# izhengfan/se2lam

Measured on NVIDIA H100. Metric: ORB keypoints/sec at 640x480 (8-level pyramid, 1000 kps/frame), higher is better.
Workload: dtype u8

## Files before the change

se2lam_b200/csrc/fast_screen.h:

```cpp
#pragma once
#include <cstdint>

#if defined(__CUDACC__)
#define SE2_HD __host__ __device__ __forceinline__
#else
#define SE2_HD inline
#endif

namespace fastpx {
SE2_HD int16_t lo16(unsigned a) { return (int16_t)(a & 0xFFFF); }
SE2_HD int16_t hi16(unsigned a) { return (int16_t)(a >> 16); }
SE2_HD unsigned pack16(int lo, int hi) { return ((unsigned)lo & 0xFFFFu) | ((unsigned)hi << 16); }
SE2_HD unsigned perm(unsigned a, unsigned b, unsigned s) {
#if defined(__CUDA_ARCH__)
    return __byte_perm(a, b, s);
#else
    const uint64_t src = ((uint64_t)b << 32) | a;
    unsigned r = 0;
    for (int i = 0; i < 4; ++i) {
        const unsigned sel = (s >> (4 * i)) & 0xF;
        unsigned byte = (unsigned)(src >> (8 * (sel & 7))) & 0xFF;
        if (sel & 8) byte = (byte & 0x80) ? 0xFF : 0x00;
        r |= byte << (8 * i);
    }
    return r;
#endif
}
SE2_HD unsigned maxs2(unsigned a, unsigned b) {
#if defined(__CUDA_ARCH__)
    return __vmaxs2(a, b);
#else
    return pack16(lo16(a) > lo16(b) ? lo16(a) : lo16(b), hi16(a) > hi16(b) ? hi16(a) : hi16(b));
#endif
}
SE2_HD unsigned mins2(unsigned a, unsigned b) {
#if defined(__CUDA_ARCH__)
    return __vmins2(a, b);
#else
    return pack16(lo16(a) < lo16(b) ? lo16(a) : lo16(b), hi16(a) < hi16(b) ? hi16(a) : hi16(b));
#endif
}
SE2_HD unsigned min3s2(unsigned a, unsigned b, unsigned c) {
#if defined(__CUDA_ARCH__)
    return __vimin3_s16x2(a, b, c);
#else
    return mins2(mins2(a, b), c);
#endif
}
SE2_HD unsigned max3s2(unsigned a, unsigned b, unsigned c) {
#if defined(__CUDA_ARCH__)
    return __vimax3_s16x2(a, b, c);
#else
    return maxs2(maxs2(a, b), c);
#endif
}
SE2_HD unsigned add2(unsigned a, unsigned b) {
#if defined(__CUDA_ARCH__)
    return __vadd2(a, b);
#else
    return pack16((lo16(a) + lo16(b)) & 0xFFFF, (hi16(a) + hi16(b)) & 0xFFFF);
#endif
}
}

namespace fastpx {

SE2_HD unsigned screen_T1(int t) { return (unsigned)(0x10000 - (257 + t)) * 0x10001u; }
SE2_HD unsigned screen_U1(int t) { return (unsigned)(256 - t) * 0x10001u; }

SE2_HD unsigned screen4(unsigned n3, unsigned s3, unsigned n2l, unsigned n2c, unsigned n2r, unsigned s2l, unsigned s2c, unsigned s2r,
                        unsigned zl, unsigned zc, unsigned zr, unsigned T1, unsigned U1) {
    const unsigned w_m3 = perm(zl, zc, 0x4321), w_p3 = perm(zc, zr, 0x6543);
    const unsigned nw_ = perm(n2l, n2c, 0x5432), ne_ = perm(n2c, n2r, 0x5432);
    const unsigned sw_ = perm(s2l, s2c, 0x5432), se_ = perm(s2c, s2r, 0x5432);
    unsigned m = 0;
#if defined(__CUDA_ARCH__)
#pragma unroll
#endif
    for (int hlf = 0; hlf < 2; ++hlf) {
        const unsigned sel = hlf ? 0x4342u : 0x4140u;
        const unsigned cb = perm(zc, 0, sel) + 0x01000100u;
        const unsigned e0 = cb - perm(s3, 0, sel), e8 = cb - perm(n3, 0, sel);
        const unsigned e4 = cb - perm(w_p3, 0, sel), e12 = cb - perm(w_m3, 0, sel);
        const unsigned e2 = cb - perm(se_, 0, sel), e10 = cb - perm(nw_, 0, sel);
        const unsigned e6 = cb - perm(ne_, 0, sel), e14 = cb - perm(sw_, 0, sel);
        const unsigned D = mins2(min3s2(maxs2(e0, e8), maxs2(e4, e12), maxs2(e2, e10)), maxs2(e6, e14));
        const unsigned B = maxs2(max3s2(mins2(e0, e8), mins2(e4, e12), mins2(e2, e10)), mins2(e6, e14));
        const unsigned r = maxs2(add2(D, T1), add2(~B, U1));
        const unsigned ok = ~r & 0x80008000u;
        m |= ((ok >> 15) & 1u) << (2 * hlf) | ((ok >> 31) & 1u) << (2 * hlf + 1);
    }
    return m;
}

SE2_HD unsigned inside_mask8(int x0, int cw) {
    const int lo = x0 < 0 ? -x0 : 0;
    const int hi = cw - x0 < 8 ? cw - x0 : 8;
    return (0xFFu << lo) & (0xFFu >> (8 - hi)) & 0xFFu;
}

SE2_HD int first_group(int shift) { return (shift + 3) >> 2; }
SE2_HD int groups_per_row(int cw, int shift) { return ((shift + 2 + cw) >> 2) - first_group(shift) + 1; }
SE2_HD int group_x0(int g, int shift) { return 4 * (g + first_group(shift)) - 3 - shift; }
struct ItemWalk {
    int y, g, dY, dG, G;
    SE2_HD void init(int tid, int nthreads, int groups) { G = groups; y = tid / G; g = tid - y * G; dY = nthreads / G; dG = nthreads - dY * G; }
    SE2_HD void next() { g += dG; y += dY; if (g >= G) { g -= G; ++y; } }
};

}
```

se2lam_b200/csrc/orb.cu:

```cuda
#include <cuda.h>

#include <algorithm>
#include <cmath>
#include <cstring>
#include <vector>

#include "blur_px.h"
#include "common.h"
#include "fast_screen.h"
#include "introselect.h"

namespace {

using se2gpu::fail;

constexpr int EDGE = 16;
constexpr int HALF_PATCH = 15;
constexpr int PATCH = 31;
constexpr int MAX_LEVELS = 16;
constexpr int FAST_THREADS = 256;
constexpr int ORB_LANES = 4;
constexpr int BLUR_WARPS = 4;
constexpr int BLUR_TH = 48;

// ... 169 lines not shown
            rowinfo[tx] = r;
            rmin = r.s0; rmax = r.s1;
        }
#pragma unroll
        for (int o = 16; o > 0; o >>= 1) { rmin = min(rmin, __shfl_xor_sync(0xffffffffu, rmin, o)); rmax = max(rmax, __shfl_xor_sync(0xffffffffu, rmax, o)); }
        if (tx == 0) { s_lo[1] = rmin; s_hi[1] = rmax; }
    }
    __syncthreads();
    const int c_min = min(min(s_cmin[0], s_cmin[1]), min(s_cmin[2], s_cmin[3])), c_max = max(max(s_cmax[0], s_cmax[1]), max(s_cmax[2], s_cmax[3]));
    const int c_lo = c_min & ~15, nvec = c_max < 0 ? 0 : (c_max - c_lo) / 16 + 1;
    const int r_lo = s_lo[1], nsr = s_hi[1] - r_lo + 1;
    if (nsr > max_rows || nvec * 16 > raw_pitch) { if (tid == 0) *d.err = 3; return; }
    const uint8_t* src = d.plain + f * d.frame_plane_bytes + S.plane_off + (size_t)EDGE * S.pitch + EDGE;
    asm volatile("griddepcontrol.wait;" ::: "memory");
    if (nvec <= 16) {
        const int v = tid & 15;
        if (v < nvec)
            for (int r = tid >> 4; r < nsr; r += 16)
                *reinterpret_cast<uint4*>(raw + r * raw_pitch + 16 * v) = __ldg(reinterpret_cast<const uint4*>(src + (size_t)(r_lo + r) * S.pitch + c_lo) + v);
    } else {
        for (int i = tid; i < nsr * nvec; i += 256) {
            const int r = i / nvec, v = i - r * nvec;
            *reinterpret_cast<uint4*>(raw + r * raw_pitch + 16 * v) = __ldg(reinterpret_cast<const uint4*>(src + (size_t)(r_lo + r) * S.pitch + c_lo) + v);
        }
    }
    int sx0[4], sx1[4], a0[4], a1[4];
    unsigned vmask = 0;
#pragma unroll
    for (int q = 0; q < 4; ++q) {
        const ResizeCol c = colinfo[4 * tx + q];
        sx0[q] = c.valid ? c.sx0 - c_lo : 0; sx1[q] = c.valid ? c.sx1 - c_lo : 0;
        a0[q] = c.a0; a1[q] = c.a1;
        vmask |= c.valid ? (0xFFu << (8 * q)) : 0u;
    }
    __syncthreads();
    unsigned wq[4], selq[4];
    bool pairq[4];
    int w0 = 0;
    bool window_ok = true;
    {
        int mn = 0x7fffffff;
#pragma unroll
        for (int q = 0; q < 4; ++q) if ((vmask >> (8 * q)) & 1u) mn = min(mn, sx0[q]);
        if (mn == 0x7fffffff) mn = 0;
        w0 = mn >> 2;
#pragma unroll
        for (int q = 0; q < 4; ++q) {
            const bool valid = (vmask >> (8 * q)) & 1u;
            const int o = valid ? sx0[q] - 4 * w0 : 0;
            if (valid && (o + 1 > 11 || (sx1[q] != sx0[q] + 1 && a1[q] != 0))) window_ok = false;
            pairq[q] = o >= 7;
            const int o2 = o - (pairq[q] ? 4 : 0);
            selq[q] = (unsigned)o2 | ((unsigned)(o2 + 1) << 4);
            wq[q] = ((unsigned)a0[q] & 0xFFFFu) | ((unsigned)a1[q] << 16);
            if (a0[q] < 0 || a1[q] < 0) window_ok = false;
        }
    }
    if (x4 < W) {
        if (window_ok) {
            for (int r = ty; r < nsr; r += 8) {
                const uint32_t* rw = reinterpret_cast<const uint32_t*>(raw + r * raw_pitch) + w0;
                const uint32_t W0 = rw[0], W1 = rw[1], W2 = rw[2];
                unsigned hq[4];
#pragma unroll
                for (int q = 0; q < 4; ++q) {
                    const unsigned bytes = __byte_perm(pairq[q] ? W1 : W0, pairq[q] ? W2 : W1, selq[q]);
                    hq[q] = __dp2a_lo(wq[q], bytes, 0u) >> 4;
                }
                *reinterpret_cast<uint2*>(hbuf + r * 128 + 4 * tx) = make_uint2(hq[0] | (hq[1] << 16), hq[2] | (hq[3] << 16));
            }
        } else {
            for (int r = ty; r < nsr; r += 8) {
                const uint8_t* rp = raw + r * raw_pitch;
                const unsigned h0 = (unsigned)((rp[sx0[0]] * a0[0] + rp[sx1[0]] * a1[0]) >> 4), h1 = (unsigned)((rp[sx0[1]] * a0[1] + rp[sx1[1]] * a1[1]) >> 4);
                const unsigned h2 = (unsigned)((rp[sx0[2]] * a0[2] + rp[sx1[2]] * a1[2]) >> 4), h3 = (unsigned)((rp[sx0[3]] * a0[3] + rp[sx1[3]] * a1[3]) >> 4);
                *reinterpret_cast<uint2*>(hbuf + r * 128 + 4 * tx) = make_uint2((h0 & 0xFFFFu) | (h1 << 16), (h2 & 0xFFFFu) | (h3 << 16));
            }
        }
    }
    __syncthreads();
    if (x4 >= L.pitch) return;
    uint8_t* plane = d.plain + f * d.frame_plane_bytes + L.plane_off;
#pragma unroll
    for (int k = 0; k < RESIZE_TR / 8; ++k) {
        const int r = ty + 8 * k, y = y0 + r;
        if (y >= H) break;
        uint32_t word = 0;
        if (x4 < W) {
            const ResizeRow ri = rowinfo[r];
            const uint2 A = *reinterpret_cast<const uint2*>(hbuf + (ri.s0 - r_lo) * 128 + 4 * tx);
            const uint2 B = *reinterpret_cast<const uint2*>(hbuf + (ri.s1 - r_lo) * 128 + 4 * tx);
            const unsigned v0 = (unsigned)((((ri.b0 * (int)(A.x & 0xFFFFu)) >> 16) + ((ri.b1 * (int)(B.x & 0xFFFFu)) >> 16) + 2) >> 2);
            const unsigned v1 = (unsigned)((((ri.b0 * (int)(A.x >> 16)) >> 16) + ((ri.b1 * (int)(B.x >> 16)) >> 16) + 2) >> 2);
            const unsigned v2 = (unsigned)((((ri.b0 * (int)(A.y & 0xFFFFu)) >> 16) + ((ri.b1 * (int)(B.y & 0xFFFFu)) >> 16) + 2) >> 2);
            const unsigned v3 = (unsigned)((((ri.b0 * (int)(A.y >> 16)) >> 16) + ((ri.b1 * (int)(B.y >> 16)) >> 16) + 2) >> 2);
            word = (v0 | (v1 << 8) | (v2 << 16) | (v3 << 24)) & vmask;
        }
        *reinterpret_cast<uint32_t*>(plane + (size_t)y * L.pitch + x4) = word;
    }
}

__device__ __forceinline__ unsigned fast_cv(int v) { return (unsigned)(256 + v) | ((unsigned)(256 - v) << 16); }
__device__ __forceinline__ unsigned fast_q(unsigned p, unsigned cv) { return p * 0xFFFFu + cv; }

__device__ __forceinline__ int fast_arc_score(const uint8_t* __restrict__ p, int pw) {
    const unsigned cv = fast_cv(p[0]);
    unsigned q[16];
    q[0] = fast_q(p[3 * pw], cv);       q[1] = fast_q(p[3 * pw + 1], cv);   q[2] = fast_q(p[2 * pw + 2], cv);    q[3] = fast_q(p[pw + 3], cv);
    q[4] = fast_q(p[3], cv);            q[5] = fast_q(p[-pw + 3], cv);      q[6] = fast_q(p[-2 * pw + 2], cv);   q[7] = fast_q(p[-3 * pw + 1], cv);
    q[8] = fast_q(p[-3 * pw], cv);      q[9] = fast_q(p[-3 * pw - 1], cv);  q[10] = fast_q(p[-2 * pw - 2], cv);  q[11] = fast_q(p[-pw - 3], cv);
    q[12] = fast_q(p[-3], cv);          q[13] = fast_q(p[pw - 3], cv);      q[14] = fast_q(p[2 * pw - 2], cv);   q[15] = fast_q(p[3 * pw - 1], cv);
    unsigned m3[16];
#pragma unroll
    for (int k = 0; k < 16; ++k) m3[k] = __vimin3_s16x2(q[k], q[(k + 1) & 15], q[(k + 2) & 15]);
    unsigned best = 0;
#pragma unroll
    for (int k = 0; k < 16; k += 2) {
        const unsigned a9 = __vimin3_s16x2(m3[k], m3[(k + 3) & 15], m3[(k + 6) & 15]);
        const unsigned b9 = __vimin3_s16x2(m3[k + 1], m3[(k + 4) & 15], m3[(k + 7) & 15]);
        best = __vimax3_s16x2(best, a9, b9);
    }
    return (int)max(best & 0xFFFFu, best >> 16) - 256;
}

struct FastMaps { CUtensorMap m[MAX_LEVELS]; };
__device__ __forceinline__ unsigned orb_smem_u32(const void* p) { return (unsigned)__cvta_generic_to_shared(p); }
__device__ __forceinline__ void orb_mbar_init(unsigned long long* bar, unsigned count) {
    asm volatile("mbarrier.init.shared::cta.b64 [%0], %1;" ::"r"(orb_smem_u32(bar)), "r"(count) : "memory");
    asm volatile("fence.mbarrier_init.release.cluster;" ::: "memory");
}
__device__ __forceinline__ bool orb_mbar_wait(unsigned long long* bar, unsigned parity) {
    const long long t0 = clock64();
    for (;;) {
        unsigned done;
        asm volatile(
            "{\n"
            ".reg .pred p;\n"
            "mbarrier.try_wait.parity.shared::cta.b64 p, [%1], %2;\n"
            "selp.u32 %0, 1, 0, p;\n"
            "}\n" : "=r"(done) : "r"(orb_smem_u32(bar)), "r"(parity) : "memory");
        if (done) return true;
        if (clock64() - t0 > 400000000LL) return false;
    }
}
__device__ __forceinline__ void orb_tma_box3(void* dst_smem, const CUtensorMap* map, int x, int y, int z, unsigned bytes, unsigned long long* bar) {
    asm volatile("mbarrier.arrive.expect_tx.shared::cta.b64 _, [%0], %1;" ::"r"(orb_smem_u32(bar)), "r"(bytes) : "memory");
    asm volatile("cp.async.bulk.tensor.3d.shared::cluster.global.tile.mbarrier::complete_tx::bytes [%0], [%1, {%2, %3, %4}], [%5];"
                 ::"r"(orb_smem_u32(dst_smem)), "l"(map), "r"(x), "r"(y), "r"(z), "r"(orb_smem_u32(bar)) : "memory");
}

template <bool TMA>
__global__ void __launch_bounds__(FAST_THREADS, TMA ? 0 : 5) orb_fast_cells(OrbDev d, const __grid_constant__ FastMaps maps) {
    extern __shared__ __align__(128) uint8_t smem_raw[];
    __shared__ int s_total, s_ncand;
    __shared__ __align__(8) unsigned long long s_bar;
    const CellGeo c = d.cells[blockIdx.x];
    const int f = blockIdx.y + d.frame0;
    CellHdr* hdr = d.hdr + (size_t)f * d.n_cells + blockIdx.x;
    const int cw = c.x1 - c.x0, ch = c.y1 - c.y0;
    if (c.skipped || cw <= 0 || ch <= 0) {
        if (threadIdx.x == 0) { hdr->n_base = 0; hdr->n_a = 0; hdr->n_b = 0; }
        return;
    }
    const LevelGeo& L = d.levels[c.level];
    const int bx0 = c.x0 - 3 + EDGE, ax0 = bx0 & (TMA ? ~15 : ~3), shift = bx0 - ax0;
    const int pw = TMA ? L.fbw : (shift + cw + 6 + 3) & ~3, pww = pw >> 2;
    const int ph = TMA ? L.fbh : ch + 6;
    uint8_t* smem = TMA ? smem_raw + ((128u - (orb_smem_u32(smem_raw) & 127u)) & 127u) : smem_raw;
    const int nbits = pw * ch, nwords = (nbits + 31) >> 5;
    const int g0 = fastpx::first_group(shift), G = fastpx::groups_per_row(cw, shift), nitems = ch * G;
    uint8_t* patch = smem;
    uint8_t* score = smem + ((pw * ph + 15) & ~15);
    uint32_t* bitmap = reinterpret_cast<uint32_t*>(score + ((pw * (ch + 2) + 15) & ~15));
    uint32_t* woff = bitmap + nwords;
    uint16_t* list = reinterpret_cast<uint16_t*>(woff + nwords);
    if (TMA) {
        if (threadIdx.x == 0) orb_mbar_init(&s_bar, 1);
        __syncthreads();
        if (threadIdx.x == 0) orb_tma_box3(patch, &maps.m[c.level], ax0, c.y0 - 3 + EDGE, f, (unsigned)(pw * ph), &s_bar);
    } else {
        const uint8_t* plane = d.plain + f * d.frame_plane_bytes + L.plane_off;
        const int by0 = c.y0 - 3 + EDGE;
        for (int i = threadIdx.x; i < pww * ph; i += FAST_THREADS) {
            const int py = i / pww, pxw = i - py * pww;
            reinterpret_cast<uint32_t*>(patch)[i] = *reinterpret_cast<const uint32_t*>(plane + (size_t)(by0 + py) * L.pitch + ax0 + 4 * pxw);
        }
    }
    constexpr int NW = FAST_THREADS / 32;
    const int lane = threadIdx.x & 31, wid = threadIdx.x >> 5;
    const uint8_t* p0 = patch + 3 * pw + 3 + shift;
    fastpx::ItemWalk first;
    first.init((int)threadIdx.x, FAST_THREADS, G);
    int thr = d.fast_th;
    for (int pass = 0; pass < 2; ++pass) {
        for (int i = threadIdx.x; i < (pw * (ch + 2) + 3) / 4; i += FAST_THREADS) reinterpret_cast<uint32_t*>(score)[i] = 0u;
        for (int i = threadIdx.x; i < nwords; i += FAST_THREADS) bitmap[i] = 0u;
        if (threadIdx.x == 0) s_ncand = 0;
        if (TMA && pass == 0 && !orb_mbar_wait(&s_bar, 0)) { *d.err = 4; return; }
        __syncthreads();
        {
            const uint32_t* pwords = reinterpret_cast<const uint32_t*>(patch);
            const unsigned T1 = fastpx::screen_T1(thr), U1 = fastpx::screen_U1(thr);
            fastpx::ItemWalk it = first;
            for (int it0 = wid * 32; it0 < nitems; it0 += NW * 32) {
                unsigned m = 0;
                const int col0 = fastpx::group_x0(it.g, shift);
                if (it.y < ch) {
                    const uint32_t* c = pwords + (it.y + 3) * pww + it.g + g0;
                    const uint32_t n3 = c[-3 * pww], s3 = c[3 * pww];
                    const uint32_t n2a = c[-2 * pww - 1], n2b = c[-2 * pww], n2c = c[-2 * pww + 1];
                    const uint32_t s2a = c[2 * pww - 1], s2b = c[2 * pww], s2c = c[2 * pww + 1];
                    const uint32_t za = c[-1], zb = c[0], zc = c[1];
                    m = fastpx::screen4(n3, s3, n2a, n2b, n2c, s2a, s2b, s2c, za, zb, zc, T1, U1) & fastpx::inside_mask8(col0, cw) & 0xFu;
                }
                const int cnt = __popc(m);
                int inc = cnt;
#pragma unroll
                for (int o = 1; o < 32; o <<= 1) { const int u = __shfl_up_sync(0xffffffffu, inc, o); if (lane >= o) inc += u; }
                const int tot = __shfl_sync(0xffffffffu, inc, 31);
                if (tot) {
                    int base = 0;
                    if (lane == 31) base = atomicAdd(&s_ncand, tot);
                    base = __shfl_sync(0xffffffffu, base, 31) + inc - cnt;
                    const int e0 = it.y * pw + col0;
                    while (m) {
                        const int j = __ffs(m) - 1;
                        m &= m - 1;
                        list[base++] = (uint16_t)(e0 + j);
                    }
                }
                it.next();
            }
        }
        __syncthreads();
        const int ncand = s_ncand;
        for (int i = threadIdx.x; i < ncand; i += FAST_THREADS) {
            const int off = list[i];
            const int m = fast_arc_score(p0 + off, pw);
            if (m > thr) score[off + pw + 1] = (uint8_t)(m - 1);
        }
        __syncthreads();
        for (int i = threadIdx.x; i < ncand; i += FAST_THREADS) {
            const int off = list[i];
            const uint8_t* q = score + off + pw + 1;
            const int sc = q[0];
            if (sc && sc > q[-pw - 1] && sc > q[-pw] && sc > q[-pw + 1] && sc > q[-1] && sc > q[1] && sc > q[pw - 1] && sc > q[pw] && sc > q[pw + 1])
                atomicOr(&bitmap[off >> 5], 1u << (off & 31));
        }
        __syncthreads();
        if (wid == 0) {
            int run = 0;
            for (int b0 = 0; b0 < nwords; b0 += 32) {
                const int v = (b0 + lane < nwords) ? __popc(bitmap[b0 + lane]) : 0;
                int inc = v;
#pragma unroll
                for (int o = 1; o < 32; o <<= 1) { const int u = __shfl_up_sync(0xffffffffu, inc, o); if (lane >= o) inc += u; }
                if (b0 + lane < nwords) woff[b0 + lane] = run + inc - v;
                run += __shfl_sync(0xffffffffu, inc, 31);
            }
            if (lane == 0) s_total = run;
        }
        __syncthreads();
        if (s_total > 3 || thr == 7) break;
        thr = 7;
        __syncthreads();
    }
    uint32_t* out = d.cand + (size_t)f * d.cand_total + c.cand_off;
    for (int j = threadIdx.x; j < nwords; j += FAST_THREADS) {
        uint32_t w = bitmap[j];
        int pos = woff[j];
        while (w) {
            const int off = j * 32 + __ffs(w) - 1;
            w &= w - 1;
            const int y = off / pw, x = off - y * pw;
            if (pos < c.cand_cap) out[pos] = ((uint32_t)score[off + pw + 1] << 24) | ((uint32_t)(c.y0 + y) << 12) | (uint32_t)(c.x0 + x);
            else *d.err = 1;
            ++pos;
        }
    }
    if (threadIdx.x == 0) { hdr->n_base = s_total; hdr->n_a = s_total; hdr->n_b = s_total; }
}

__device__ __forceinline__ int fast_arc_score_qr(const uint8_t* __restrict__ p, int pw, int t) {
    const int v = p[0];
    const int c0 = v - p[3 * pw], c8 = v - p[-3 * pw];
    bool dk = (c0 > t) | (c8 > t), br = (c0 < -t) | (c8 < -t);
    if (!(dk | br)) return 0;
    const int c4 = v - p[3], c12 = v - p[-3];
    dk &= (c4 > t) | (c12 > t); br &= (c4 < -t) | (c12 < -t);
    if (!(dk | br)) return 0;
    const int c2 = v - p[2 * pw + 2], c10 = v - p[-2 * pw - 2];
    dk &= (c2 > t) | (c10 > t); br &= (c2 < -t) | (c10 < -t);
    if (!(dk | br)) return 0;
    const int c6 = v - p[-2 * pw + 2], c14 = v - p[2 * pw - 2];
    dk &= (c6 > t) | (c14 > t); br &= (c6 < -t) | (c14 < -t);
    if (!(dk | br)) return 0;
#define SE2_PK(dv) ((static_cast<unsigned>(dv) & 0xFFFFu) | (static_cast<unsigned>(-(dv)) << 16))
    unsigned q[16];
    q[0] = SE2_PK(c0);   q[1] = SE2_PK(v - p[3 * pw + 1]);    q[2] = SE2_PK(c2);    q[3] = SE2_PK(v - p[pw + 3]);
    q[4] = SE2_PK(c4);   q[5] = SE2_PK(v - p[-pw + 3]);       q[6] = SE2_PK(c6);    q[7] = SE2_PK(v - p[-3 * pw + 1]);
    q[8] = SE2_PK(c8);   q[9] = SE2_PK(v - p[-3 * pw - 1]);   q[10] = SE2_PK(c10);  q[11] = SE2_PK(v - p[-pw - 3]);
    q[12] = SE2_PK(c12); q[13] = SE2_PK(v - p[pw - 3]);       q[14] = SE2_PK(c14);  q[15] = SE2_PK(v - p[3 * pw - 1]);
#undef SE2_PK
    unsigned m3[16];
#pragma unroll
    for (int k = 0; k < 16; ++k) m3[k] = __vimin3_s16x2(q[k], q[(k + 1) & 15], q[(k + 2) & 15]);
    unsigned best = 0x80008000u;
#pragma unroll
    for (int k = 0; k < 16; k += 2) {
        const unsigned a9 = __vimin3_s16x2(m3[k], m3[(k + 3) & 15], m3[(k + 6) & 15]);
        const unsigned b9 = __vimin3_s16x2(m3[k + 1], m3[(k + 4) & 15], m3[(k + 7) & 15]);
        best = __vimax3_s16x2(best, a9, b9);
    }
    const int mdark = static_cast<short>(best & 0xFFFFu), mbright = static_cast<short>(best >> 16);
    return max(mdark, mbright);
}

__global__ void __launch_bounds__(FAST_THREADS) orb_fast_cells_big(OrbDev d) {
    extern __shared__ uint8_t smem[];
    __shared__ int s_total;
    const CellGeo c = d.cells[blockIdx.x];
    const int f = blockIdx.y + d.frame0;
    CellHdr* hdr = d.hdr + (size_t)f * d.n_cells + blockIdx.x;
    const int cw = c.x1 - c.x0, ch = c.y1 - c.y0;
    if (c.skipped || cw <= 0 || ch <= 0) {
        if (threadIdx.x == 0) { hdr->n_base = 0; hdr->n_a = 0; hdr->n_b = 0; }
        return;
    }
    const LevelGeo& L = d.levels[c.level];
    const uint8_t* plane = d.plain + f * d.frame_plane_bytes + L.plane_off;
    const int bx0 = c.x0 - 3 + EDGE, by0 = c.y0 - 3 + EDGE;
    const int ax0 = bx0 & ~3, shift = bx0 - ax0;
    const int ph = ch + 6, sw = cw + 2, sh = ch + 2;
    const int pww = (shift + cw + 6 + 3) >> 2, pw = pww * 4;
    uint8_t* patch = smem;
    uint8_t* score = smem + ((pw * ph + 15) & ~15);
    const int nseg = (cw + 31) >> 5, nchunk = ch * nseg;
    int* cnt = reinterpret_cast<int*>(score + ((sw * sh + 15) & ~15));
    for (int i = threadIdx.x; i < pww * ph; i += FAST_THREADS) {
        const int py = i / pww, pxw = i - py * pww;
        reinterpret_cast<uint32_t*>(patch)[i] = *reinterpret_cast<const uint32_t*>(plane + (size_t)(by0 + py) * L.pitch + ax0 + 4 * pxw);
    }
    constexpr int NW = FAST_THREADS / 32;
    const int lane = threadIdx.x & 31, wid = threadIdx.x >> 5;
    const uint8_t* p0 = patch + 3 * pw + 3 + shift;
    int thr = d.fast_th;
    unsigned long long keepmask = 0;
    for (int pass = 0; pass < 2; ++pass) {
        for (int i = threadIdx.x; i < (sw * sh + 3) / 4; i += FAST_THREADS) reinterpret_cast<uint32_t*>(score)[i] = 0u;
        __syncthreads();
        for (int cidx = wid; cidx < nchunk; cidx += NW) {
            const int y = cidx / nseg, x = (cidx - y * nseg) * 32 + lane;
            if (x < cw) {
                const int m = fast_arc_score_qr(p0 + y * pw + x, pw, thr);
                if (m > thr) score[(y + 1) * sw + (x + 1)] = (uint8_t)(m - 1);
            }
        }
        __syncthreads();
        keepmask = 0;
        int t = 0;
        for (int cidx = wid; cidx < nchunk; cidx += NW, ++t) {
            const int y = cidx / nseg, x = (cidx - y * nseg) * 32 + lane;
            bool keep = false;
            if (x < cw) {
                const uint8_t* q = score + (y + 1) * sw + (x + 1);
                const int s = q[0];
                if (s) keep = s > q[-sw - 1] && s > q[-sw] && s > q[-sw + 1] && s > q[-1] && s > q[1] && s > q[sw - 1] && s > q[sw] && s > q[sw + 1];
            }
            const unsigned bal = __ballot_sync(0xffffffffu, keep);
            if (lane == 0) cnt[cidx] = __popc(bal);
            if (keep && t < 64) keepmask |= 1ull << t;
        }
        __syncthreads();
        if (wid == 0) {
            int run = 0;
            for (int b0 = 0; b0 < nchunk; b0 += 32) {
                const int v = (b0 + lane < nchunk) ? cnt[b0 + lane] : 0;
                int inc = v;
#pragma unroll
                for (int o = 1; o < 32; o <<= 1) { const int u = __shfl_up_sync(0xffffffffu, inc, o); if (lane >= o) inc += u; }
                if (b0 + lane < nchunk) cnt[b0 + lane] = run + inc - v;
                run += __shfl_sync(0xffffffffu, inc, 31);
            }
            if (lane == 0) s_total = run;
        }
        __syncthreads();
        if (s_total > 3 || thr == 7) break;
        thr = 7;
        __syncthreads();
    }
    uint32_t* out = d.cand + (size_t)f * d.cand_total + c.cand_off;
    int t = 0;
    for (int cidx = wid; cidx < nchunk; cidx += NW, ++t) {
        const int y = cidx / nseg, x = (cidx - y * nseg) * 32 + lane;
        bool keep;
        int s = 0;
        if (t < 64) {
            keep = (keepmask >> t) & 1ull;
        } else {
            keep = false;
            if (x < cw) {
                const uint8_t* q = score + (y + 1) * sw + (x + 1);
                s = q[0];
                if (s) keep = s > q[-sw - 1] && s > q[-sw] && s > q[-sw + 1] && s > q[-1] && s > q[1] && s > q[sw - 1] && s > q[sw] && s > q[sw + 1];
            }
        }
        const unsigned bal = __ballot_sync(0xffffffffu, keep);
        if (keep) {
            s = score[(y + 1) * sw + (x + 1)];
            const int pos = cnt[cidx] + __popc(bal & ((1u << lane) - 1));
            if (pos < c.cand_cap) out[pos] = ((uint32_t)s << 24) | ((uint32_t)(c.y0 + y) << 12) | (uint32_t)(c.x0 + x);
            else *d.err = 1;
        }
    }
    if (threadIdx.x == 0) { hdr->n_base = s_total; hdr->n_a = s_total; hdr->n_b = s_total; }
}

constexpr int SEL_STAGE = 12288;
constexpr int SEL_THREADS = 512;
__global__ void __launch_bounds__(SEL_THREADS) orb_select(OrbDev d) {
    extern __shared__ uint32_t sbuf[];
    __shared__ int wq[SEL_THREADS / 32][128];
    constexpr int NW = SEL_THREADS / 32;
    const int lane = threadIdx.x & 31, wid = threadIdx.x >> 5;
    const int level = blockIdx.x, f = blockIdx.y + d.frame0;
    const LevelGeo& L = d.levels[level];
    const int nCells = L.nCells;
    const int cap = 2 * L.nDesired + 4 * nCells + 64;
    uint32_t* lbuf = sbuf;
    int* nTotal = (int*)(sbuf + cap);
    int* nToRetain = nTotal + nCells;
    int* kept = nToRetain + nCells;
    int* koff = kept + nCells;
// ... 212 lines not shown
                if (v0 + k <= vm) { colsum += p[k] + m[k]; m01 += (v0 + k) * (p[k] - m[k]); }
        }
        m10 = u * colsum;
    }
#pragma unroll
    for (int o = 16; o > 0; o >>= 1) { m10 += __shfl_xor_sync(0xffffffffu, m10, o); m01 += __shfl_xor_sync(0xffffffffu, m01, o); }
    const float angle = fast_atan2_deg((float)m01, (float)m10);
    const float factorPI = (float)(M_PI / 180.f);
    const float ang = __fmul_rn(angle, factorPI);
    double sd, cd;
    sincos((double)ang, &sd, &cd);
    const float a = (float)cd, b = (float)sd;
    const uint8_t* bc = d.blurred + base;
    unsigned val = 0;
    int o0[8], o1[8];
#pragma unroll
    for (int k = 0; k < 8; ++k) {
        const float4 pt = patf[k * 32 + lane];
        const float x0 = pt.x, y0 = pt.y, x1 = pt.z, y1 = pt.w;
        const int r0 = __float2int_rn(__fadd_rn(__fmul_rn(x0, b), __fmul_rn(y0, a)));
        const int c0 = __float2int_rn(__fsub_rn(__fmul_rn(x0, a), __fmul_rn(y0, b)));
        const int r1 = __float2int_rn(__fadd_rn(__fmul_rn(x1, b), __fmul_rn(y1, a)));
        const int c1 = __float2int_rn(__fsub_rn(__fmul_rn(x1, a), __fmul_rn(y1, b)));
        o0[k] = r0 * L.pitch + c0; o1[k] = r1 * L.pitch + c1;
    }
    int t0[8], t1[8];
#pragma unroll
    for (int k = 0; k < 8; ++k) { t0[k] = bc[o0[k]]; t1[k] = bc[o1[k]]; }
#pragma unroll
    for (int k = 0; k < 8; ++k) val |= (unsigned)(t0[k] < t1[k]) << k;
    unsigned w = val;
    w |= __shfl_down_sync(0xffffffffu, val, 1) << 8;
    w |= __shfl_down_sync(0xffffffffu, val, 2) << 16;
    w |= __shfl_down_sync(0xffffffffu, val, 3) << 24;
    const size_t oslot = (size_t)f * d.nfeatures + slot;
    if ((lane & 3) == 0) reinterpret_cast<unsigned*>(desc + oslot * 32)[lane >> 2] = w;
    if (lane == 0) {
        se2gpu_keypoint kp;
        kp.x = level ? __fmul_rn((float)x, L.scale) : (float)x;
        kp.y = level ? __fmul_rn((float)y, L.scale) : (float)y;
        kp.size = L.kp_size; kp.angle = angle; kp.response = (float)score; kp.octave = level; kp.class_id = -1;
        kps[oslot] = kp;
    }
}

inline int cv_round_f(float v) { return (int)lrintf(v); }

}

struct se2gpu_orb {
    int device = 0, nfeatures = 0, nlevels = 0, fast_th = 20, max_w = 0, max_h = 0, max_batch = 0;
    double scaleFactor = 1.2;
    std::vector<float> mvScaleFactor, mvInvScaleFactor;
    std::vector<int> mnFeaturesPerLevel;
    int cur_w = -1, cur_h = -1;
    std::vector<LevelGeo> levels;
    std::vector<CellGeo> cells;
    std::vector<TileGeo> tiles;
    size_t fast_smem = 0, select_smem = 0, resize_w_smem = 0;
    int resize_rows = 0, resize_raw_pitch = 0;
    bool fast_big = false;
    bool fast_tma = false;
    size_t fast_tma_smem = 0;
    FastMaps fast_maps{};
    bool und_on = false;
    float und_K[9] = {}, und_D[14] = {};
    int und_nd = 0, und_w = 0, und_h = 0;
    short2* d_und_m1 = nullptr; uint16_t* d_und_m2 = nullptr; size_t und_cap = 0;
    size_t cap_plane = 0, cap_cand = 0, cap_cells = 0, cap_tiles = 0, cap_tab = 0, cap_lkp = 0;
    OrbDev d{};
    LevelGeo* d_levels = nullptr; CellGeo* d_cells = nullptr; TileGeo* d_tiles = nullptr; int* d_itab = nullptr; short* d_stab = nullptr;

    uint8_t* d_in = nullptr; se2gpu_keypoint* d_kps = nullptr; uint8_t* d_desc = nullptr; int* d_counts = nullptr;
    std::vector<void*> bufs;
    int last_n = 0;
    se2gpu::Profiler prof;
    cudaStream_t side = nullptr;
    cudaEvent_t ev_pyr = nullptr, ev_blur = nullptr, ev_l1 = nullptr;
    cudaStream_t pipe[ORB_LANES] = {};
    int* pin_counts = nullptr; se2gpu_keypoint* pin_kps = nullptr; uint8_t* pin_desc = nullptr;
    struct Pending { bool on = false; int n = 0, lanes = 0; bool pipelined = false; se2gpu_keypoint* kps = nullptr; uint8_t* desc = nullptr; int* counts = nullptr;
                     se2gpu_keypoint* out_kps = nullptr; uint8_t* out_desc = nullptr; int* out_counts = nullptr; } pend;
    se2gpu_orb* twin = nullptr;
    int submit_next = 0, wait_next = 0, in_flight = 0;
    int create_args[8] = {};
};

namespace {

int build_geometry(se2gpu_orb* h, int w, int hgt, bool dry, size_t* plane_bytes, size_t* cand_total, size_t* n_cells,
                   size_t* n_tiles, size_t* tab_total, size_t* max_fast_smem, size_t* max_select_smem,
                   std::vector<LevelGeo>* Lv, std::vector<CellGeo>* Cv, std::vector<TileGeo>* Tv, bool* fast_big_out = nullptr,
                   size_t* fast_tma_smem_out = nullptr) {
    (void)dry;
    const int nl = h->nlevels;
    std::vector<LevelGeo> L(nl);
    std::vector<CellGeo> C;
    std::vector<TileGeo> T;
    size_t poff = 0, coff = 0, toff = 0, fsm = 0, ssm = 0, fsm_big = 0, fsm_tma = 0;
    bool fast_big = false;
    bool tma_ok = true;
    int kp_off = 0;
    const float imageRatio = (float)w / (float)hgt;
    for (int l = 0; l < nl; ++l) {
        LevelGeo& g = L[l];
        const float scale = h->mvInvScaleFactor[l];
        g.w = cv_round_f((float)w * scale); g.h = cv_round_f((float)hgt * scale);
        if (g.w < 2 * EDGE + 7 || g.h < 2 * EDGE + 7) return fail(SE2GPU_ERR_INVALID, "level %d of a %dx%d frame is %dx%d: too small for the 16 px border", l, w, hgt, g.w, g.h);
        if (g.w + 2 * EDGE > 4095 || g.h + 2 * EDGE > 4095) return fail(SE2GPU_ERR_CAPACITY, "frames wider/taller than 4063 px are not supported");
        g.pitch = (g.w + 2 * EDGE + 31) & ~31;
        g.plane_off = poff;
        poff += (size_t)g.pitch * (g.h + 2 * EDGE);
        poff = (poff + 255) & ~(size_t)255;
        g.nDesired = h->mnFeaturesPerLevel[l];
        g.cols = (int)sqrtf((float)g.nDesired / (5 * imageRatio));
        g.rows = (int)(imageRatio * g.cols);
        if (g.cols < 1 || g.rows < 1) return fail(SE2GPU_ERR_INVALID, "level %d has a %dx%d cell grid (nfeatures too small): undefined in the reference", l, g.cols, g.rows);
        const int minB = EDGE, maxBX = g.w - EDGE, maxBY = g.h - EDGE;
        const int W = maxBX - minB, H = maxBY - minB;
        const int cellW = (int)ceilf((float)W / g.cols), cellH = (int)ceilf((float)H / g.rows);
        g.nCells = g.rows * g.cols;
        g.nfeaturesCell = (int)ceilf((float)g.nDesired / g.nCells);
        g.cell_base = (int)C.size();
        g.kp_off = kp_off; g.kp_cap = g.nDesired; kp_off += g.nDesired;
        g.scale = h->mvScaleFactor[l];
        g.kp_size = (float)(int)(PATCH * h->mvScaleFactor[l]);
        g.tab_off = (int)toff; toff += (size_t)g.w + g.h;
        std::vector<int> iniXCol(g.cols, 0);
        const size_t first_cell = C.size();
        int max_cw = 0, max_ch = 0;
        float hY = cellH + 6;
        for (int i = 0; i < g.rows; ++i) {
            const float iniY = minB + i * cellH - 3;
            bool rowSkipped = false;
            if (i == g.rows - 1) { hY = maxBY + 3 - iniY; if (hY <= 0) rowSkipped = true; }
            float hX = cellW + 6;
            for (int j = 0; j < g.cols; ++j) {
                CellGeo c{};
                c.level = l;
                if (rowSkipped) { c.skipped = 1; C.push_back(c); continue; }
                float iniX;
                if (i == 0) { iniX = minB + j * cellW - 3; iniXCol[j] = (int)iniX; } else iniX = iniXCol[j];
                if (j == g.cols - 1) { hX = maxBX + 3 - iniX; if (hX <= 0) { c.skipped = 1; C.push_back(c); continue; } }
                const int r0 = (int)iniY, r1 = (int)(iniY + hY), c0 = (int)iniX, c1 = (int)(iniX + hX);
                if (r1 > g.h || c1 > g.w || r0 < 0 || c0 < 0) return fail(SE2GPU_ERR_INVALID, "cell grid of level %d leaves the image (the reference asserts here)", l);
                c.x0 = c0 + 3; c.x1 = c1 - 3; c.y0 = r0 + 3; c.y1 = r1 - 3;
                const int cw = std::max(c.x1 - c.x0, 0), chh = std::max(c.y1 - c.y0, 0);
                c.cand_off = (int)coff;
                c.cand_cap = ((cw + 1) / 2) * ((chh + 1) / 2) + 8;
                coff += c.cand_cap;
                if (cw > 0 && chh > 0) {
                    max_cw = std::max(max_cw, ((c.x0 - 3 + EDGE) & 15) + cw); max_ch = std::max(max_ch, chh);
                    const size_t pwb = (size_t)((cw + 6 + 3 + 3) / 4 + 1) * 4;
                    const size_t nwords = (pwb * chh + 31) / 32;
                    if (pwb * (chh + 6) > 65535) fast_big = true;
                    fsm = std::max(fsm, ((pwb * (chh + 6) + 15) & ~(size_t)15) + ((pwb * (chh + 2) + 15) & ~(size_t)15) + nwords * 8 + (size_t)cw * chh * 2 + 64);
                    const size_t nchunk = (size_t)chh * ((cw + 31) / 32);
                    fsm_big = std::max(fsm_big, ((pwb * (chh + 6) + 15) & ~(size_t)15) + (((size_t)(cw + 2) * (chh + 2) + 15) & ~(size_t)15) + nchunk * 4 + 64);
                }
                C.push_back(c);
            }
        }
        g.fbw = (max_cw + 6 + 15) & ~15; g.fbh = max_ch + 6;
        if (max_cw > 0) {
            if (g.fbw > 256 || g.fbh > 256 || (size_t)g.fbw * g.fbh > 65535) tma_ok = false;
            for (size_t ci = first_cell; ci < C.size(); ++ci) {
                const int cw = C[ci].x1 - C[ci].x0, chh = C[ci].y1 - C[ci].y0;
                if (C[ci].skipped || cw <= 0 || chh <= 0) continue;
                const size_t pw = (size_t)g.fbw, nwords = (pw * chh + 31) / 32;
                fsm_tma = std::max(fsm_tma, (size_t)128 + ((pw * g.fbh + 15) & ~(size_t)15) + ((pw * (chh + 2) + 15) & ~(size_t)15) + nwords * 8 + (size_t)cw * chh * 2 + 64);
            }
        }
        ssm = std::max(ssm, (size_t)(2 * g.nDesired + 4 * g.nCells + 64) * 4 + (size_t)g.nCells * 16 + (size_t)SEL_STAGE * 4);
        g.tile_base = (int)T.size();
        g.blur_strips = std::max(2, (g.h + BLUR_TH - 1) / BLUR_TH);
        g.blur_th = ((g.h + g.blur_strips - 1) / g.blur_strips + 12) / 7 * 7 - 6;
        for (int it = 0; it < g.blur_strips * (g.pitch / 8); it += 32) T.push_back(TileGeo{l, it / (g.pitch / 8), it % (g.pitch / 8)});
    }
    *plane_bytes = poff; *cand_total = coff; *n_cells = C.size(); *n_tiles = T.size(); *tab_total = toff;
    if (fsm > 227 * 1024) fast_big = true;
    *max_fast_smem = fast_big ? fsm_big : fsm; *max_select_smem = ssm;
    if (fast_big_out) *fast_big_out = fast_big;
    if (fast_tma_smem_out) *fast_tma_smem_out = (tma_ok && !fast_big && fsm_tma <= 227 * 1024) ? fsm_tma : 0;
    if (Lv) *Lv = L;
    if (Cv) *Cv = C;
    if (Tv) *Tv = T;
    return SE2GPU_OK;
}

typedef CUresult (*EncodeTiledFn)(CUtensorMap*, CUtensorMapDataType, cuuint32_t, void*, const cuuint64_t*, const cuuint64_t*, const cuuint32_t*,
                                  const cuuint32_t*, CUtensorMapInterleave, CUtensorMapSwizzle, CUtensorMapL2promotion, CUtensorMapFloatOOBfill);
EncodeTiledFn tensor_map_encoder() {
    static EncodeTiledFn fn = [] {
        void* p = nullptr;
        cudaDriverEntryPointQueryResult q = cudaDriverEntryPointSymbolNotFound;
        if (cudaGetDriverEntryPoint("cuTensorMapEncodeTiled", &p, cudaEnableDefault, &q) != cudaSuccess || q != cudaDriverEntryPointSuccess) { cudaGetLastError(); p = nullptr; }
        return (EncodeTiledFn)p;
    }();
    return fn;
}

constexpr int BLUR_SPLIT = 1;
constexpr int PIPE_CHUNKS = 4, PIPE_FIRST_PCT = 50, SUBMIT_CHUNKS = 1;

bool encode_fast_maps(se2gpu_orb* h, size_t frame_plane_bytes) {
    EncodeTiledFn enc = tensor_map_encoder();
    if (!enc || (frame_plane_bytes & 15)) return false;
    for (int l = 0; l < h->nlevels; ++l) {
        const LevelGeo& g = h->levels[l];
        if (g.fbw <= 6) { memset(&h->fast_maps.m[l], 0, sizeof(CUtensorMap)); continue; }
        const cuuint64_t gdim[3] = {(cuuint64_t)g.pitch, (cuuint64_t)(g.h + 2 * EDGE), (cuuint64_t)h->max_batch};
        const cuuint64_t gstr[2] = {(cuuint64_t)g.pitch, (cuuint64_t)frame_plane_bytes};
        const cuuint32_t box[3] = {(cuuint32_t)g.fbw, (cuuint32_t)g.fbh, 1u};
        const cuuint32_t estr[3] = {1u, 1u, 1u};
        void* base = h->d.plain + g.plane_off;
        if (((uintptr_t)base & 15) || (g.pitch & 15)) return false;
        if (enc(&h->fast_maps.m[l], CU_TENSOR_MAP_DATA_TYPE_UINT8, 3, base, gdim, gstr, box, estr, CU_TENSOR_MAP_INTERLEAVE_NONE,
                CU_TENSOR_MAP_SWIZZLE_NONE, CU_TENSOR_MAP_L2_PROMOTION_L2_128B, CU_TENSOR_MAP_FLOAT_OOB_FILL_NONE) != CUDA_SUCCESS) return false;
    }
    return true;
}

int set_geometry(se2gpu_orb* h, int w, int hgt, cudaStream_t s) {
    if (w == h->cur_w && hgt == h->cur_h) return SE2GPU_OK;
    size_t pb, ct, nc, nt, tt, fsm, ssm, fsm_tma = 0;
    bool big = false;
    int rc = build_geometry(h, w, hgt, false, &pb, &ct, &nc, &nt, &tt, &fsm, &ssm, &h->levels, &h->cells, &h->tiles, &big, &fsm_tma);
    if (rc != SE2GPU_OK) return rc;
    if (pb > h->cap_plane || ct > h->cap_cand || nc > h->cap_cells || nt > h->cap_tiles || tt > h->cap_tab)
        return fail(SE2GPU_ERR_CAPACITY, "frame %dx%d exceeds the capacity this extractor was created with (%dx%d)", w, hgt, h->max_w, h->max_h);
    if (fsm > 227 * 1024) return fail(SE2GPU_ERR_CAPACITY, "a FAST cell of a %dx%d frame needs %zu B of shared memory", w, hgt, fsm);
    std::vector<int> itab(tt, 0);
    std::vector<short> stab(2 * tt, 0);
    for (int l = 1; l < h->nlevels; ++l) {
        const LevelGeo& g = h->levels[l];
        const LevelGeo& sg = h->levels[l - 1];
        const double scale_x = 1. / ((double)g.w / sg.w), scale_y = 1. / ((double)g.h / sg.h);
        int* xofs = itab.data() + g.tab_off; int* yofs = xofs + g.w;
        short* ialpha = stab.data() + 2 * (size_t)g.tab_off; short* ibeta = ialpha + 2 * g.w;
        for (int dx = 0; dx < g.w; ++dx) {
            float fx = (float)((dx + 0.5) * scale_x - 0.5);
            int sx = (int)floorf(fx);
            fx -= sx;
            if (sx < 0) { fx = 0; sx = 0; }
            if (sx >= sg.w - 1) { fx = 0; sx = sg.w - 1; }
            xofs[dx] = sx;
            ialpha[2 * dx] = (short)std::min(std::max(cv_round_f((1.f - fx) * 2048.f), -32768), 32767);
            ialpha[2 * dx + 1] = (short)std::min(std::max(cv_round_f(fx * 2048.f), -32768), 32767);
        }
        for (int dy = 0; dy < g.h; ++dy) {
            float fy = (float)((dy + 0.5) * scale_y - 0.5);
            int sy = (int)floorf(fy);
            fy -= sy;
            yofs[dy] = sy;
            ibeta[2 * dy] = (short)cv_round_f((1.f - fy) * 2048.f);
            ibeta[2 * dy + 1] = (short)cv_round_f(fy * 2048.f);
        }
    }
    SE2_CUDA(cudaMemcpyAsync(h->d_levels, h->levels.data(), sizeof(LevelGeo) * h->levels.size(), cudaMemcpyHostToDevice, s));
    SE2_CUDA(cudaMemcpyAsync(h->d_cells, h->cells.data(), sizeof(CellGeo) * h->cells.size(), cudaMemcpyHostToDevice, s));
    SE2_CUDA(cudaMemcpyAsync(h->d_tiles, h->tiles.data(), sizeof(TileGeo) * h->tiles.size(), cudaMemcpyHostToDevice, s));
    SE2_CUDA(cudaMemcpyAsync(h->d_itab, itab.data(), sizeof(int) * itab.size(), cudaMemcpyHostToDevice, s));
    SE2_CUDA(cudaMemcpyAsync(h->d_stab, stab.data(), sizeof(short) * stab.size(), cudaMemcpyHostToDevice, s));
    SE2_CUDA(cudaStreamSynchronize(s));
    h->fast_smem = fsm; h->select_smem = ssm; h->fast_big = big;
    {
        double ratio = 1.0;
        for (size_t l = 1; l < h->levels.size(); ++l)
            ratio = std::max(ratio, std::max((double)h->levels[l - 1].w / h->levels[l].w, (double)h->levels[l - 1].h / h->levels[l].h));
        h->resize_rows = (int)ceil(RESIZE_TR * ratio) + 4;
        h->resize_raw_pitch = (((int)ceil(128 * ratio) + 4 + 15 + 15) / 16) * 16;
        h->resize_w_smem = (size_t)h->resize_rows * (128 * sizeof(uint16_t) + h->resize_raw_pitch) + 16;
        if (h->resize_w_smem > 200 * 1024) return fail(SE2GPU_ERR_CAPACITY, "scale factor %.3f needs %zu B of shared memory in orb_resize_w", ratio, h->resize_w_smem);
        SE2_CUDA(cudaFuncSetAttribute(orb_resize_w, cudaFuncAttributeMaxDynamicSharedMemorySize, (int)h->resize_w_smem));
    }
    SE2_CUDA(cudaFuncSetAttribute(orb_fast_cells_big, cudaFuncAttributeMaxDynamicSharedMemorySize, (int)std::max<size_t>(fsm, 1024)));
    SE2_CUDA(cudaFuncSetAttribute(orb_fast_cells<false>, cudaFuncAttributeMaxDynamicSharedMemorySize, (int)std::max<size_t>(fsm, 1024)));
    h->fast_tma = fsm_tma > 0 && encode_fast_maps(h, pb);
    h->fast_tma_smem = fsm_tma;
    if (h->fast_tma) SE2_CUDA(cudaFuncSetAttribute(orb_fast_cells<true>, cudaFuncAttributeMaxDynamicSharedMemorySize, (int)std::max<size_t>(fsm_tma, 1024)));
    SE2_CUDA(cudaFuncSetAttribute(orb_select, cudaFuncAttributeMaxDynamicSharedMemorySize, (int)std::max<size_t>(ssm, 1024)));
    OrbDev& d = h->d;
    d.n_cells = (int)h->cells.size(); d.n_tiles = (int)h->tiles.size();
    d.frame_plane_bytes = pb; d.cand_total = ct;
    int lk = 0; for (auto& g : h->levels) lk += g.kp_cap;
    d.lkp_total = lk;
    h->cur_w = w; h->cur_h = hgt;
    return SE2GPU_OK;
}

int build_undistort_map(const float* K, const float* dist, int nd, int w, int hgt, std::vector<short2>& m1, std::vector<uint16_t>& m2) {
    double A[9], D[14] = {0};
    for (int i = 0; i < 9; ++i) A[i] = K[i];
    for (int i = 0; i < nd; ++i) D[i] = dist[i];
    m1.resize((size_t)w * hgt); m2.resize((size_t)w * hgt);
    const int stripe = std::min(std::max(1, 4096 / std::max(w, 1)), hgt);
    for (int y0 = 0; y0 < hgt; y0 += stripe) {
        double M[9], inv[9] = {1, 0, 0, 0, 1, 0, 0, 0, 1};
        for (int i = 0; i < 9; ++i) M[i] = A[i];
        M[5] = A[5] - y0;
        for (int c = 0; c < 3; ++c) {
            int piv = c;
            for (int r = c + 1; r < 3; ++r) if (std::fabs(M[r * 3 + c]) > std::fabs(M[piv * 3 + c])) piv = r;
            if (std::fabs(M[piv * 3 + c]) < 2.220446049250313e-14) return fail(SE2GPU_ERR_INVALID, "singular camera matrix");
            if (piv != c) for (int q = 0; q < 3; ++q) { std::swap(M[c * 3 + q], M[piv * 3 + q]); std::swap(inv[c * 3 + q], inv[piv * 3 + q]); }
            const double dneg = -1 / M[c * 3 + c];
            for (int r = c + 1; r < 3; ++r) {
                const double al = M[r * 3 + c] * dneg;
                for (int q = c + 1; q < 3; ++q) M[r * 3 + q] += al * M[c * 3 + q];
                for (int q = 0; q < 3; ++q) inv[r * 3 + q] += al * inv[c * 3 + q];
            }
        }
        for (int r = 2; r >= 0; --r)
            for (int q = 0; q < 3; ++q) {
                double acc = inv[r * 3 + q];
                for (int t = r + 1; t < 3; ++t) acc -= M[r * 3 + t] * inv[t * 3 + q];
                inv[r * 3 + q] = acc / M[r * 3 + r];
            }
        const int rows = std::min(stripe, hgt - y0);
        for (int i = 0; i < rows; ++i) {
            double X = i * inv[1] + inv[2], Y = i * inv[4] + inv[5], Wc = i * inv[7] + inv[8];
            short2* o1 = m1.data() + (size_t)(y0 + i) * w;
            uint16_t* o2 = m2.data() + (size_t)(y0 + i) * w;
// ... 409 lines not shown
```

Measured before the change: 93.83 million.

## Vectorize FAST non-max suppression into per-row bitmaps with SIMD compares

Replaces the per-candidate 3x3 NMS and atomicOr bitmap with a dense SIMD pass over the score plane that produces 32-bit row-aligned masks per thread. A block-level prefix sum built from per-warp sums replaces the single-warp serial scan and the woff array. Candidate compaction now uses four ballots instead of a shuffle scan, which removes the serial ffs loop. This cuts atomics, scattered shared-memory reads and one barrier. In exchange the NMS work now covers every pixel rather than only candidates, and the score plane is shifted to offset NMS_X0 with extra padding.

```diff
diff --git a/se2lam_b200/csrc/fast_screen.h b/se2lam_b200/csrc/fast_screen.h
--- a/se2lam_b200/csrc/fast_screen.h
+++ b/se2lam_b200/csrc/fast_screen.h
@@ -108,4 +108,55 @@
     SE2_HD void next() { g += dG; y += dY; if (g >= G) { g -= G; ++y; } }
 };
 
+constexpr int NMS_X0 = 4;
+SE2_HD int nms_plane_bytes(int pw, int ch) { return pw * (ch + 2) + 32; }
+SE2_HD int nms_words_per_row(int cw) { return (cw + 31) >> 5; }
+SE2_HD unsigned nms_row_mask(int k, int cw) { const int n = cw - 32 * k; return n >= 32 ? 0xFFFFFFFFu : (1u << n) - 1u; }
+
+SE2_HD unsigned nms32(const uint32_t* u, const uint32_t* c, const uint32_t* d) {
+    unsigned c3e[10], c3o[10];
+    unsigned r[4];
+#if defined(__CUDA_ARCH__)
+#pragma unroll
+#endif
+    for (int j = 0; j < 10; ++j) {
+        const unsigned ua = u[j], ca = c[j], da = d[j];
+        if (j > 0) c3e[j] = max3s2(perm(ua, 0, 0x4240), perm(ca, 0, 0x4240), perm(da, 0, 0x4240));
+        if (j < 9) c3o[j] = max3s2(perm(ua, 0, 0x4341), perm(ca, 0, 0x4341), perm(da, 0, 0x4341));
+    }
+#if defined(__CUDA_ARCH__)
+#pragma unroll
+#endif
+    for (int g = 0; g < 8; ++g) {
+        const int j = g + 1;
+        const unsigned ua = u[j], ca = c[j], da = d[j];
+        const unsigned ce = perm(ca, 0, 0x4240), co = perm(ca, 0, 0x4341);
+        const unsigned ve = maxs2(perm(ua, 0, 0x4240), perm(da, 0, 0x4240));
+        const unsigned vo = maxs2(perm(ua, 0, 0x4341), perm(da, 0, 0x4341));
+        const unsigned ne = max3s2(perm(c3o[j - 1], c3o[j], 0x5432), ve, c3o[j]);
+        const unsigned no = max3s2(c3e[j], vo, perm(c3e[j], c3e[j + 1], 0x5432));
+        const unsigned te = ce + 0x00FF00FFu - ne, to = co + 0x00FF00FFu - no;
+        const unsigned bytes = perm(te, to, 0x7351);
+        if (g & 1) {
+            r[g >> 1] = (r[g >> 1] + (bytes << 4)) * 0x01020408u;
+        } else {
+            r[g >> 1] = bytes;
+        }
+    }
+    return perm(perm(r[0], r[1], 0x7373), perm(r[2], r[3], 0x7373), 0x5410);
 }
+
+struct WordRun {
+    int w, w1, y, k, wpr;
+    SE2_HD void init(int tid, int nthreads, int ch, int words_per_row) {
+        wpr = words_per_row;
+        const int nw = ch * wpr, q = (nw + nthreads - 1) / nthreads;
+        w = tid * q < nw ? tid * q : nw;
+        w1 = w + q < nw ? w + q : nw;
+        y = w / wpr; k = w - y * wpr;
+    }
+    SE2_HD bool more() const { return w < w1; }
+    SE2_HD void next() { ++w; if (++k == wpr) { k = 0; ++y; } }
+};
+
+}
diff --git a/se2lam_b200/csrc/orb.cu b/se2lam_b200/csrc/orb.cu
--- a/se2lam_b200/csrc/orb.cu
+++ b/se2lam_b200/csrc/orb.cu
@@ -345,7 +345,7 @@
 template <bool TMA>
 __global__ void __launch_bounds__(FAST_THREADS, TMA ? 0 : 5) orb_fast_cells(OrbDev d, const __grid_constant__ FastMaps maps) {
     extern __shared__ __align__(128) uint8_t smem_raw[];
-    __shared__ int s_total, s_ncand;
+    __shared__ int s_ncand, s_wsum[FAST_THREADS / 32];
     __shared__ __align__(8) unsigned long long s_bar;
     const CellGeo c = d.cells[blockIdx.x];
     const int f = blockIdx.y + d.frame0;
@@ -360,13 +360,12 @@
     const int pw = TMA ? L.fbw : (shift + cw + 6 + 3) & ~3, pww = pw >> 2;
     const int ph = TMA ? L.fbh : ch + 6;
     uint8_t* smem = TMA ? smem_raw + ((128u - (orb_smem_u32(smem_raw) & 127u)) & 127u) : smem_raw;
-    const int nbits = pw * ch, nwords = (nbits + 31) >> 5;
     const int g0 = fastpx::first_group(shift), G = fastpx::groups_per_row(cw, shift), nitems = ch * G;
+    const int wpr = fastpx::nms_words_per_row(cw);
     uint8_t* patch = smem;
     uint8_t* score = smem + ((pw * ph + 15) & ~15);
-    uint32_t* bitmap = reinterpret_cast<uint32_t*>(score + ((pw * (ch + 2) + 15) & ~15));
-    uint32_t* woff = bitmap + nwords;
-    uint16_t* list = reinterpret_cast<uint16_t*>(woff + nwords);
+    uint32_t* bitmap = reinterpret_cast<uint32_t*>(score + ((fastpx::nms_plane_bytes(pw, ch) + 15) & ~15));
+    uint16_t* list = reinterpret_cast<uint16_t*>(bitmap + ch * wpr);
     if (TMA) {
         if (threadIdx.x == 0) orb_mbar_init(&s_bar, 1);
         __syncthreads();
@@ -384,10 +383,12 @@
     const uint8_t* p0 = patch + 3 * pw + 3 + shift;
     fastpx::ItemWalk first;
     first.init((int)threadIdx.x, FAST_THREADS, G);
+    fastpx::WordRun words;
+    words.init((int)threadIdx.x, FAST_THREADS, ch, wpr);
     int thr = d.fast_th;
+    int total = 0, pos0 = 0;
     for (int pass = 0; pass < 2; ++pass) {
-        for (int i = threadIdx.x; i < (pw * (ch + 2) + 3) / 4; i += FAST_THREADS) reinterpret_cast<uint32_t*>(score)[i] = 0u;
-        for (int i = threadIdx.x; i < nwords; i += FAST_THREADS) bitmap[i] = 0u;
+        for (int i = threadIdx.x; i < pw * (ch + 2) / 4; i += FAST_THREADS) reinterpret_cast<uint32_t*>(score)[i] = 0u;
         if (threadIdx.x == 0) s_ncand = 0;
         if (TMA && pass == 0 && !orb_mbar_wait(&s_bar, 0)) { *d.err = 4; return; }
         __syncthreads();
@@ -406,21 +407,19 @@
                     const uint32_t za = c[-1], zb = c[0], zc = c[1];
                     m = fastpx::screen4(n3, s3, n2a, n2b, n2c, s2a, s2b, s2c, za, zb, zc, T1, U1) & fastpx::inside_mask8(col0, cw) & 0xFu;
                 }
-                const int cnt = __popc(m);
-                int inc = cnt;
-#pragma unroll
-                for (int o = 1; o < 32; o <<= 1) { const int u = __shfl_up_sync(0xffffffffu, inc, o); if (lane >= o) inc += u; }
-                const int tot = __shfl_sync(0xffffffffu, inc, 31);
+                const unsigned b0 = __ballot_sync(0xffffffffu, m & 1u), b1 = __ballot_sync(0xffffffffu, m & 2u);
+                const unsigned b2 = __ballot_sync(0xffffffffu, m & 4u), b3 = __ballot_sync(0xffffffffu, m & 8u);
+                const int n0 = __popc(b0), n01 = n0 + __popc(b1), n012 = n01 + __popc(b2), tot = n012 + __popc(b3);
                 if (tot) {
                     int base = 0;
-                    if (lane == 31) base = atomicAdd(&s_ncand, tot);
-                    base = __shfl_sync(0xffffffffu, base, 31) + inc - cnt;
+                    if (lane == 0) base = atomicAdd(&s_ncand, tot);
+                    base = __shfl_sync(0xffffffffu, base, 0);
+                    const unsigned lt = (1u << lane) - 1u;
                     const int e0 = it.y * pw + col0;
-                    while (m) {
-                        const int j = __ffs(m) - 1;
-                        m &= m - 1;
-                        list[base++] = (uint16_t)(e0 + j);
-                    }
+                    if (m & 1u) list[base + __popc(b0 & lt)] = (uint16_t)e0;
+                    if (m & 2u) list[base + n0 + __popc(b1 & lt)] = (uint16_t)(e0 + 1);
+                    if (m & 4u) list[base + n01 + __popc(b2 & lt)] = (uint16_t)(e0 + 2);
+                    if (m & 8u) list[base + n012 + __popc(b3 & lt)] = (uint16_t)(e0 + 3);
                 }
                 it.next();
             }
@@ -430,48 +429,42 @@
         for (int i = threadIdx.x; i < ncand; i += FAST_THREADS) {
             const int off = list[i];
             const int m = fast_arc_score(p0 + off, pw);
-            if (m > thr) score[off + pw + 1] = (uint8_t)(m - 1);
+            if (m > thr) score[off + pw + fastpx::NMS_X0] = (uint8_t)(m - 1);
         }
         __syncthreads();
-        for (int i = threadIdx.x; i < ncand; i += FAST_THREADS) {
-            const int off = list[i];
-            const uint8_t* q = score + off + pw + 1;
-            const int sc = q[0];
-            if (sc && sc > q[-pw - 1] && sc > q[-pw] && sc > q[-pw + 1] && sc > q[-1] && sc > q[1] && sc > q[pw - 1] && sc > q[pw] && sc > q[pw + 1])
-                atomicOr(&bitmap[off >> 5], 1u << (off & 31));
-        }
+        int nkp = 0;
+        for (fastpx::WordRun r = words; r.more(); r.next()) {
+            const uint32_t* u = reinterpret_cast<const uint32_t*>(score) + r.y * pww + 8 * r.k;
+            const unsigned bits = fastpx::nms32(u, u + pww, u + 2 * pww) & fastpx::nms_row_mask(r.k, cw);
+            bitmap[r.w] = bits;
+            nkp += __popc(bits);
+        }
+        int inc = nkp;
+#pragma unroll
+        for (int o = 1; o < 32; o <<= 1) { const int u = __shfl_up_sync(0xffffffffu, inc, o); if (lane >= o) inc += u; }
+        if (lane == 31) s_wsum[wid] = inc;
         __syncthreads();
-        if (wid == 0) {
-            int run = 0;
-            for (int b0 = 0; b0 < nwords; b0 += 32) {
-                const int v = (b0 + lane < nwords) ? __popc(bitmap[b0 + lane]) : 0;
-                int inc = v;
-#pragma unroll
-                for (int o = 1; o < 32; o <<= 1) { const int u = __shfl_up_sync(0xffffffffu, inc, o); if (lane >= o) inc += u; }
-                if (b0 + lane < nwords) woff[b0 + lane] = run + inc - v;
-                run += __shfl_sync(0xffffffffu, inc, 31);
-            }
-            if (lane == 0) s_total = run;
-        }
-        __syncthreads();
-        if (s_total > 3 || thr == 7) break;
+        total = 0; pos0 = inc - nkp;
+#pragma unroll
+        for (int w = 0; w < NW; ++w) { const int v = s_wsum[w]; total += v; if (w < wid) pos0 += v; }
+        if (total > 3 || thr == 7) break;
         thr = 7;
-        __syncthreads();
     }
     uint32_t* out = d.cand + (size_t)f * d.cand_total + c.cand_off;
-    for (int j = threadIdx.x; j < nwords; j += FAST_THREADS) {
-        uint32_t w = bitmap[j];
-        int pos = woff[j];
-        while (w) {
-            const int off = j * 32 + __ffs(w) - 1;
-            w &= w - 1;
-            const int y = off / pw, x = off - y * pw;
-            if (pos < c.cand_cap) out[pos] = ((uint32_t)score[off + pw + 1] << 24) | ((uint32_t)(c.y0 + y) << 12) | (uint32_t)(c.x0 + x);
+    int pos = pos0;
+    for (fastpx::WordRun r = words; r.more(); r.next()) {
+        uint32_t bits = bitmap[r.w];
+        const uint8_t* srow = score + (r.y + 1) * pw + fastpx::NMS_X0 + 32 * r.k;
+        const uint32_t yx = ((uint32_t)(c.y0 + r.y) << 12) | (uint32_t)(c.x0 + 32 * r.k);
+        while (bits) {
+            const int i = __ffs(bits) - 1;
+            bits &= bits - 1;
+            if (pos < c.cand_cap) out[pos] = ((uint32_t)srow[i] << 24) | (yx + i);
             else *d.err = 1;
             ++pos;
         }
     }
-    if (threadIdx.x == 0) { hdr->n_base = s_total; hdr->n_a = s_total; hdr->n_b = s_total; }
+    if (threadIdx.x == 0) { hdr->n_base = total; hdr->n_a = total; hdr->n_b = total; }
 }
 
 __device__ __forceinline__ int fast_arc_score_qr(const uint8_t* __restrict__ p, int pw, int t) {
@@ -990,9 +983,9 @@
                 if (cw > 0 && chh > 0) {
                     max_cw = std::max(max_cw, ((c.x0 - 3 + EDGE) & 15) + cw); max_ch = std::max(max_ch, chh);
                     const size_t pwb = (size_t)((cw + 6 + 3 + 3) / 4 + 1) * 4;
-                    const size_t nwords = (pwb * chh + 31) / 32;
+                    const size_t bitmap = (size_t)chh * fastpx::nms_words_per_row(cw) * 4;
                     if (pwb * (chh + 6) > 65535) fast_big = true;
-                    fsm = std::max(fsm, ((pwb * (chh + 6) + 15) & ~(size_t)15) + ((pwb * (chh + 2) + 15) & ~(size_t)15) + nwords * 8 + (size_t)cw * chh * 2 + 64);
+                    fsm = std::max(fsm, ((pwb * (chh + 6) + 15) & ~(size_t)15) + (((size_t)fastpx::nms_plane_bytes((int)pwb, chh) + 15) & ~(size_t)15) + bitmap + (size_t)cw * chh * 2 + 64);
                     const size_t nchunk = (size_t)chh * ((cw + 31) / 32);
                     fsm_big = std::max(fsm_big, ((pwb * (chh + 6) + 15) & ~(size_t)15) + (((size_t)(cw + 2) * (chh + 2) + 15) & ~(size_t)15) + nchunk * 4 + 64);
                 }
@@ -1005,8 +998,8 @@
             for (size_t ci = first_cell; ci < C.size(); ++ci) {
                 const int cw = C[ci].x1 - C[ci].x0, chh = C[ci].y1 - C[ci].y0;
                 if (C[ci].skipped || cw <= 0 || chh <= 0) continue;
-                const size_t pw = (size_t)g.fbw, nwords = (pw * chh + 31) / 32;
-                fsm_tma = std::max(fsm_tma, (size_t)128 + ((pw * g.fbh + 15) & ~(size_t)15) + ((pw * (chh + 2) + 15) & ~(size_t)15) + nwords * 8 + (size_t)cw * chh * 2 + 64);
+                const size_t pw = (size_t)g.fbw, bitmap = (size_t)chh * fastpx::nms_words_per_row(cw) * 4;
+                fsm_tma = std::max(fsm_tma, (size_t)128 + ((pw * g.fbh + 15) & ~(size_t)15) + (((size_t)fastpx::nms_plane_bytes(g.fbw, chh) + 15) & ~(size_t)15) + bitmap + (size_t)cw * chh * 2 + 64);
             }
         }
         ssm = std::max(ssm, (size_t)(2 * g.nDesired + 4 * g.nCells + 64) * 4 + (size_t)g.nCells * 16 + (size_t)SEL_STAGE * 4);
```

After: 100.1 million, median of 6. 1.07x the previous value.
